# kazuto1011/dusty-gan

Measured on NVIDIA B200. Metric: chamfer_pairs_per_s, higher is better.
Workload: dtype f32

## Files before the change

### dusty-gan_b200/csrc/chamfer.cu

```cuda
#include <algorithm>

#include "common.cuh"

namespace dusty {
namespace chamfer {

constexpr int TPB = 256;
constexpr int TILE = 2048;
constexpr int CHUNK = 32;

struct Params {
  const float4* scanX;
  const float4* scanY;
  long long strideX, strideY;
  int countX, countY;
  int paddedX, paddedY;
  int row_begin, row_stride;
  int symmetric, mirror, compact_rows;
  float* M;
  long long ldm;
  float* dist1; float* dist2;
  int* idx1; int* idx2;
  const int2* metaX; const int2* metaY;
  const float4* boxX; const float4* boxY;
// ... 22 lines not shown

__device__ __forceinline__ float search_window(float ax, float ay, float az, float cur) {
  const float an = fmaf(az, az, fmaf(ax, ax, ay * ay));
  return fmaf(2.86102295e-6f , an + fmaxf(cur + an, 0.0f), 1e-36f);
}

template <bool WANT_INDEX>
__device__ __forceinline__ void warp_tile_exact_min(const float4* tp, int npairs, float ax, float ay, float az, int lane,
                                                    float& best, int& best_pos) {
  const f32x2 ax2 = pack2(ax, ax), ay2 = pack2(ay, ay), az2 = pack2(az, az);
  float e = __int_as_float(0x7f800000);
  int ei = 0x7fffffff;
  for (int q = lane; q < npairs; q += 32) {
    const float4 q0 = tp[2 * q], q1 = tp[2 * q + 1];
    const f32x2 dx = sub2(pack2(q0.x, q0.y), ax2);
    const f32x2 dy = sub2(pack2(q0.z, q0.w), ay2);
    const f32x2 dz = sub2(pack2(q1.x, q1.y), az2);
    float lo, hi;
    unpack2(fma2(dz, dz, fma2(dx, dx, mul2(dy, dy))), lo, hi);
    if (WANT_INDEX) {
      if (lo < e) { e = lo; ei = 2 * q; }
      if (hi < e) { e = hi; ei = 2 * q + 1; }
    } else {
      e = min3(e, lo, hi);
    }
  }
  float m = e;
  #pragma unroll
  for (int o = 16; o > 0; o >>= 1) m = fminf(m, __shfl_xor_sync(0xffffffffu, m, o));
  best = m;
  if (WANT_INDEX) {
    const bool mine = e == m && ei != 0x7fffffff;
    const unsigned key = mine ? (unsigned)ei : 0x7fffffffu;
    const unsigned kmin = __reduce_min_sync(0xffffffffu, key);
    const unsigned who = __ballot_sync(0xffffffffu, mine && key == kmin);
    best_pos = who ? __shfl_sync(0xffffffffu, ei, __ffs(who) - 1) : 0x7fffffff;
  }
}

template <bool WANT_INDEX>
__device__ __forceinline__ void warp_cloud_exact_min(const float4* cloud, int nchunks, const float4* boxes, float thr,
                                                     float ax, float ay, float az, int lane, const int* perm, float& best,
                                                     int& best_pos) {
  const f32x2 ax2 = pack2(ax, ax), ay2 = pack2(ay, ay), az2 = pack2(az, az);
  float e = __int_as_float(0x7f800000);
  int ei = 0x7fffffff;
  for (int ch = lane; ch < nchunks; ch += 32) {
    if (boxes != nullptr) {
      const float4 bl = boxes[2 * ch], bh = boxes[2 * ch + 1];
      const float gx = max3(0.0f, bl.x - ax, ax - bh.x), gy = max3(0.0f, bl.y - ay, ay - bh.y), gz = max3(0.0f, bl.z - az, az - bh.z);
      if (bl.w == 0.0f && fmaf(gz, gz, fmaf(gx, gx, __fmul_rn(gy, gy))) > thr) continue;
    }
    const float4* cp = cloud + (long long)ch * CHUNK;
    #pragma unroll 4
    for (int k = 0; k < CHUNK / 2; ++k) {
      const float4 q0 = cp[2 * k], q1 = cp[2 * k + 1];
      const f32x2 dx = sub2(pack2(q0.x, q0.y), ax2);
      const f32x2 dy = sub2(pack2(q0.z, q0.w), ay2);
      const f32x2 dz = sub2(pack2(q1.x, q1.y), az2);
      float lo, hi;
      unpack2(fma2(dz, dz, fma2(dx, dx, mul2(dy, dy))), lo, hi);
      if (WANT_INDEX) {
        const int i0 = ch * CHUNK + 2 * k;
        if (lo < e || (lo == e && ei != 0x7fffffff && (perm ? perm[i0] < perm[ei] : i0 < ei))) { e = lo; ei = i0; }
        if (hi < e || (hi == e && ei != 0x7fffffff && (perm ? perm[i0 + 1] < perm[ei] : i0 + 1 < ei))) { e = hi; ei = i0 + 1; }
      } else {
        e = min3(e, lo, hi);
      }
    }
  }
  float m = e;
  #pragma unroll
  for (int o = 16; o > 0; o >>= 1) m = fminf(m, __shfl_xor_sync(0xffffffffu, m, o));
  best = m;
  if (WANT_INDEX) {
    const bool mine = e == m && ei != 0x7fffffff;
    const unsigned key = mine ? (unsigned)(perm ? perm[ei] : ei) : 0x7fffffffu;
    const unsigned kmin = __reduce_min_sync(0xffffffffu, key);
    const unsigned who = __ballot_sync(0xffffffffu, mine && key == kmin);
    best_pos = who ? __shfl_sync(0xffffffffu, ei, __ffs(who) - 1) : 0x7fffffff;
  }
}

__device__ __forceinline__ void emit_entry(const Params& p, int ci, int cj, double S0, double S1) {
  const float v = (float)(S0 / (double)p.countX) + (float)(S1 / (double)p.countY);
  if (p.M) {
    p.M[(long long)(p.compact_rows ? (int)blockIdx.y : ci) * p.ldm + cj] = v;
    if (p.symmetric && p.mirror && ci != cj) p.M[(long long)cj * p.ldm + ci] = v;
  }
  if (p.keys) {
    const int gi = p.offX + ci, gj = p.offY + cj;
    if (gi != gj) {
      const unsigned long long vb = (unsigned long long)__float_as_uint(v) << 32;
      atomicMin(p.keys + gj, vb | (unsigned)gi);
      atomicMin(p.keys + gi, vb | (unsigned)gj);
      const int lo = min(gi, gj), hi = max(gi, gj);
      if (lo < p.n_ref && hi >= p.n_ref) {
        atomicMin(p.keys + p.n_total + hi, vb | (unsigned)lo);
        atomicMin(p.keys + 2 * (long long)p.n_total + lo, vb | (unsigned)hi);
      }
    }
  }
}

template <int R, bool MATRIX, bool MERGED, int NT = TPB>
__global__ void __launch_bounds__(NT, R >= 8 ? 512 / NT : (R == 4 ? 3 : 4)) nn_kernel(const Params p) {
  static_assert(!MERGED || MATRIX, "merged origins are a matrix front end layout");
  extern __shared__ __align__(128) unsigned char smem_raw[];
  float4* const tiles = reinterpret_cast<float4*>(smem_raw);
  __shared__ uint64_t bars[2];
  __shared__ double red[NT / 32];

  constexpr int RB = NT * R;
  constexpr int CH = (NT < TPB && !MERGED) ? CHUNK / 2 : CHUNK;
  constexpr int PR = CH / 2;
  const int tid = threadIdx.x;
  const int lane = tid & 31;

  int ci, cj;
  int dir_only = -1, rb_only = 0;
  if (MATRIX) {
    ci = p.row_begin + blockIdx.y * p.row_stride;
    cj = blockIdx.x;
    if (p.symmetric && cj < ci) return;
  } else {
    ci = cj = blockIdx.y;
    dir_only = blockIdx.z;
    rb_only = blockIdx.x;
    const int rows_here = dir_only == 0 ? p.countX : p.countY;
    if (rb_only >= (rows_here + RB - 1) / RB) return;
  }
  const float4* const sx = p.scanX + (long long)ci * p.strideX;
  const float4* const sy = p.scanY + (long long)cj * p.strideY;

  int2 mx = make_int2(p.countX, 1), my = make_int2(p.countY, 1);
  if (MERGED) { mx = p.metaX[ci]; my = p.metaY[cj]; }
#define K_ROW(r) (MERGED ? rb * RB + (tid >> 5) * (32 * R) + (r) * 32 + lane : rb * RB + (r) * NT + tid)
#define K_countX (MERGED ? mx.x : p.countX)
#define K_countY (MERGED ? my.x : p.countY)
#define K_paddedX (MERGED ? (mx.x + CHUNK - 1) / CHUNK * CHUNK : p.paddedX)
#define K_paddedY (MERGED ? (my.x + CHUNK - 1) / CHUNK * CHUNK : p.paddedY)

  const int ntX = (K_paddedX + TILE - 1) / TILE, ntY = (K_paddedY + TILE - 1) / TILE;
  const int nrbX = (K_countX + RB - 1) / RB, nrbY = (K_countY + RB - 1) / RB;
  const int seg0 = nrbX * ntY;
  int pos_begin, pos_end;
  if (MATRIX) { pos_begin = 0; pos_end = seg0 + nrbY * ntX; }
  else if (dir_only == 0) { pos_begin = rb_only * ntY; pos_end = pos_begin + ntY; }
  else { pos_begin = seg0 + rb_only * ntX; pos_end = pos_begin + ntX; }

  const int tstride = (R >= 8 && NT == TPB) ? TILE : min(TILE, max(p.paddedX, p.paddedY));
  if (tid == 0) { mbar_init(&bars[0], 1); mbar_init(&bars[1], 1); mbar_fence_init(); }
  __syncthreads();

  auto issue = [&](int pos, int buf) {
    int dir, t;
    if (pos < seg0) { dir = 0; t = pos % ntY; } else { dir = 1; t = (pos - seg0) % ntX; }
    const float4* src = (dir == 0 ? sy : sx) + (long long)t * TILE;
    const int padded = dir == 0 ? K_paddedY : K_paddedX;
    const int npts = min(TILE, padded - t * TILE);
    mbar_expect_tx(&bars[buf], (uint32_t)npts * 16u);
    bulk_g2s(tiles + buf * tstride, src, (uint32_t)npts * 16u, &bars[buf]);
  };
  if (tid == 0) issue(pos_begin, 0);

  f32x2 nax[R], nay[R], naz[R];
  float eb[R];
  int ei[R];
  float cur[R], sec[R];
  int cid[R];
// ... 128 lines not shown
        while (flagged) {
          const int src = __ffs(flagged) - 1;
          flagged &= flagged - 1;
          float m;
          int mi = 0;
          warp_tile_exact_min<!MATRIX>(tp, nch * PR, __shfl_sync(0xffffffffu, ax, src), __shfl_sync(0xffffffffu, ay, src),
                                       __shfl_sync(0xffffffffu, az, src), lane, m, mi);
          if (lane == src) {
            if (MATRIX) {
              eb[r] = fminf(eb[r], m);
            } else if (mi != 0x7fffffff) {
              mi += t * TILE;
              if (m < eb[r] || (m == eb[r] && mi < ei[r])) { eb[r] = m; ei[r] = mi; }
            }
          }
        }
      }
    }

    }

    if (MERGED && t == nt - 1 && rb * RB + (tid >> 5) * (32 * R) < rowcount) {
      const float4* const cand = dir == 0 ? sy : sx;
      #pragma unroll
      for (int r = 0; r < R; ++r) {
        float ax, ay, az, dummy;
        unpack2(nax[r], ax, dummy); unpack2(nay[r], ay, dummy); unpack2(naz[r], az, dummy);
        ax *= -0.5f; ay *= -0.5f; az *= -0.5f;
        const bool live = K_ROW(r) < rowcount;
        float e = __int_as_float(0x7f800000);
        if (live && cur[r] < __int_as_float(0x7f800000)) {
          const f32x2 ax2 = pack2(ax, ax), ay2 = pack2(ay, ay), az2 = pack2(az, az);
          const float4* cp = cand + (long long)cid[r] * CHUNK;
          #pragma unroll 4
          for (int k = 0; k < CHUNK / 2; ++k) {
            const float4 q0 = cp[2 * k], q1 = cp[2 * k + 1];
            const f32x2 dx = sub2(pack2(q0.x, q0.y), ax2);
            const f32x2 dy = sub2(pack2(q0.z, q0.w), ay2);
            const f32x2 dz = sub2(pack2(q1.x, q1.y), az2);
            float lo, hi;
            unpack2(fma2(dz, dz, fma2(dx, dx, mul2(dy, dy))), lo, hi);
            e = min3(e, lo, hi);
          }
        }
        eb[r] = e;
        const bool near_tie = live && sec[r] <= cur[r] + search_window(ax, ay, az, cur[r]);
        unsigned flagged = __ballot_sync(0xffffffffu, near_tie);
        while (flagged) {
          const int src = __ffs(flagged) - 1;
          flagged &= flagged - 1;
          float m;
          int mi;
          warp_cloud_exact_min<false>(cand, scanpadded / CHUNK, nullptr, 0.0f, __shfl_sync(0xffffffffu, ax, src),
                                      __shfl_sync(0xffffffffu, ay, src), __shfl_sync(0xffffffffu, az, src), lane, nullptr, m, mi);
          if (lane == src) eb[r] = fminf(eb[r], m);
        }
      }
    }

    if (t == nt - 1) {
      #pragma unroll
      for (int r = 0; r < R; ++r) {
        const int row = K_ROW(r);
        if (row < rowcount) {
          if (MATRIX) {
            if (MERGED) dsum += (row == rowcount - 1 ? (double)(dir == 0 ? mx.y : my.y) : 1.0) * (double)eb[r];
            else dsum += (double)eb[r];
          } else {
            float* dist = dir == 0 ? p.dist1 : p.dist2;
            int* idx = dir == 0 ? p.idx1 : p.idx2;
            const long long o = (long long)ci * rowcount + row;
            dist[o] = eb[r];
            if (idx) idx[o] = ei[r] == 0x7fffffff ? 0 : ei[r];
          }
        }
      }
    }
    if (MATRIX && pos == seg0 - 1) { S0 = block_sum<NT>(dsum, red); dsum = 0.0; }
    __syncthreads();
  }

  if (MATRIX) {
    const double S1 = block_sum<NT>(dsum, red);
    if (tid == 0) emit_entry(p, ci, cj, S0, S1);
  }
}

#undef K_ROW
#undef K_countX
#undef K_countY
#undef K_paddedX
#undef K_paddedY

__global__ void __launch_bounds__(256) prep_kernel(const float* __restrict__ xyz, long long clouds, int count,
                                                   int padded, float4* __restrict__ out) {
  const long long half = padded / 2;
  const long long g = (long long)blockIdx.x * blockDim.x + threadIdx.x;
  if (g >= clouds * half) return;
  const long long c = g / half;
  const int q = (int)(g - c * half);
  const float nan = __int_as_float(0x7fc00000);
  float v[2][4];
  #pragma unroll
  for (int s = 0; s < 2; ++s) {
    const int pt = 2 * q + s;
    if (pt < count) {
      const float* src = xyz + (c * count + pt) * 3;
      const float x = src[0], y = src[1], z = src[2];
      v[s][0] = x; v[s][1] = y; v[s][2] = z;
      v[s][3] = fmaf(z, z, fmaf(x, x, y * y));
    } else {
      v[s][0] = v[s][1] = v[s][2] = v[s][3] = nan;
    }
  }
  out[g * 2] = make_float4(v[0][0], v[1][0], v[0][1], v[1][1]);
  out[g * 2 + 1] = make_float4(v[0][2], v[1][2], v[0][3], v[1][3]);
}

__global__ void __launch_bounds__(256) prep_merge_kernel(const float* __restrict__ xyz, int count, long long stride,
                                                         float4* __restrict__ out, int2* __restrict__ meta) {
  __shared__ int wsum[8];
  const long long c = blockIdx.x;
  const int tid = threadIdx.x, lane = tid & 31, warp = tid >> 5;
  const float* src = xyz + c * count * 3;
  float* dst = reinterpret_cast<float*>(out + c * stride);
  const int per = (count + 255) / 256;
  const int begin = min(tid * per, count), end = min(begin + per, count);
  int mine = 0;
  for (int i = begin; i < end; ++i) mine += (src[3 * i] != 0.0f) || (src[3 * i + 1] != 0.0f) || (src[3 * i + 2] != 0.0f);
  int inc = mine;
  #pragma unroll
  for (int o = 1; o < 32; o <<= 1) { const int t = __shfl_up_sync(0xffffffffu, inc, o); if (lane >= o) inc += t; }
  if (lane == 31) wsum[warp] = inc;
  __syncthreads();
  int before = 0, total = 0;
  #pragma unroll
  for (int w = 0; w < 8; ++w) { if (w < warp) before += wsum[w]; total += wsum[w]; }
  auto put = [&](int pos, float x, float y, float z, float n) {
    float* q = dst + (size_t)(pos >> 1) * 8 + (pos & 1);
    q[0] = x; q[2] = y; q[4] = z; q[6] = n;
  };
  int pos = before + inc - mine;
  for (int i = begin; i < end; ++i) {
    const float x = src[3 * i], y = src[3 * i + 1], z = src[3 * i + 2];
    if (x != 0.0f || y != 0.0f || z != 0.0f) put(pos++, x, y, z, fmaf(z, z, fmaf(x, x, y * y)));
  }
  const int zeros = count - total;
  const int kept = total + (zeros > 0 ? 1 : 0);
  if (tid == 0) {
    if (zeros > 0) put(total, 0.0f, 0.0f, 0.0f, 0.0f);
    meta[c] = make_int2(kept, zeros > 0 ? zeros : 1);
  }
  const float nan = __int_as_float(0x7fc00000);
  const int padded = (kept + CHUNK - 1) / CHUNK * CHUNK;
  for (int i = kept + tid; i < padded; i += 256) put(i, nan, nan, nan, nan);
}

constexpr int SORT_CAP = 32768;
constexpr int SORT_TPB = 1024;
constexpr int WALK_BLOCKS = SORT_CAP / CHUNK / 32;

__device__ __forceinline__ unsigned spread7(unsigned v) {
  v &= 0x7fu;
  v = (v | (v << 4)) & 0x070fu;
  v = (v | (v << 2)) & 0x1333u;
  v = (v | (v << 1)) & 0x1555u;
  return v;
// ... 649 lines not shown
```

### dusty-gan_b200/csrc/chamfer_pair.cuh

```cuda
constexpr int PAIR_CAP = 2048;
constexpr int PAIR_NW = 8;

__global__ void __launch_bounds__(PAIR_NW * 32, 3) nn_pair_split_kernel(const Params p) {
  constexpr int SUB = 8;
  constexpr int GR = 32;
  extern __shared__ __align__(128) unsigned char smem_raw[];
  __shared__ uint64_t bar;
  __shared__ double tsum[2 * (PAIR_CAP / GR)];
  __shared__ int next_task;
  const int tid = threadIdx.x, lane = tid & 31;
  const int h = lane >> 4, l16 = lane & 15;

  const int ci = p.row_begin + blockIdx.y * p.row_stride;
  const int cj = blockIdx.x;
  if (p.symmetric && cj < ci) return;

  const int2 mx = p.metaX[ci], my = p.metaY[cj];
  const int padX = (mx.x + CHUNK - 1) / CHUNK * CHUNK, padY = (my.x + CHUNK - 1) / CHUNK * CHUNK;
  float4* const sX = reinterpret_cast<float4*>(smem_raw);
  float4* const sY = sX + p.paddedX;
  float4* const bX = sY + p.paddedY;
  float4* const bY = bX + p.paddedX / CHUNK * 2;
  if (tid == 0) {
    mbar_init(&bar, 1);
    mbar_fence_init();
    next_task = 0;
    const uint32_t bytes = (uint32_t)(padX + padY) * 16u + (uint32_t)(padX / CHUNK + padY / CHUNK) * 32u;
    mbar_expect_tx(&bar, bytes);
    bulk_g2s(sX, p.scanX + (long long)ci * p.strideX, (uint32_t)padX * 16u, &bar);
    bulk_g2s(sY, p.scanY + (long long)cj * p.strideY, (uint32_t)padY * 16u, &bar);
    bulk_g2s(bX, p.boxX + (long long)ci * (p.paddedX / CHUNK * 2), (uint32_t)(padX / CHUNK) * 32u, &bar);
    bulk_g2s(bY, p.boxY + (long long)cj * (p.paddedY / CHUNK * 2), (uint32_t)(padY / CHUNK) * 32u, &bar);
  }
  __syncthreads();
  mbar_wait(&bar, 0);

  const int ngX = (mx.x + GR - 1) / GR, ngY = (my.x + GR - 1) / GR;
  const float inf = __int_as_float(0x7f800000);

  for (;;) {
    int task = 0;
    if (lane == 0) task = atomicAdd(&next_task, 1);
    task = __shfl_sync(0xffffffffu, task, 0);
    if (task >= ngX + ngY) break;
    const int dir = task >= ngX;
    const int g = dir ? task - ngX : task;
    const float4* const rows = dir ? sY : sX;
    const float4* const cand = dir ? sX : sY;
    const float4* const rbox = dir ? bY : bX;
    const float4* const cbox = dir ? bX : bY;
    const int rowcount = dir ? my.x : mx.x;
    const int nch = (dir ? padX : padY) / CHUNK;

    f32x2 nax[2], nay[2], naz[2];
    float cur[2], sec[2];
    int cid[2];
    float rx[2], ry[2], rz[2];
    #pragma unroll
    for (int j = 0; j < 2; ++j) {
      const int row = g * GR + j * 16 + l16;
      const int rr = row < rowcount ? row : 0;
      const float* f = reinterpret_cast<const float*>(rows + (rr >> 1) * 2) + (rr & 1);
      rx[j] = f[0]; ry[j] = f[2]; rz[j] = f[4];
      const float mx2 = -2.0f * rx[j], my2 = -2.0f * ry[j], mz2 = -2.0f * rz[j];
      nax[j] = pack2(mx2, mx2); nay[j] = pack2(my2, my2); naz[j] = pack2(mz2, mz2);
      cur[j] = sec[j] = inf; cid[j] = 0;
    }
    const float oax = h ? rx[1] : rx[0], oay = h ? ry[1] : ry[0], oaz = h ? rz[1] : rz[0];
    const float an = fmaf(oaz, oaz, fmaf(oax, oax, oay * oay));
    const int orow = g * GR + lane;
    float ubr = orow < rowcount ? inf : -1.0f;
    float gl0, gl1, gl2, gh0, gh1, gh2;
    {
      const float4 bl = rbox[2 * g], bh = rbox[2 * g + 1];
      gl0 = bl.x; gl1 = bl.y; gl2 = bl.z; gh0 = bh.x; gh1 = bh.y; gh2 = bh.z;
      if (bl.w != 0.0f) {
        gl0 = fminf(gl0, 0.0f); gl1 = fminf(gl1, 0.0f); gl2 = fminf(gl2, 0.0f);
        gh0 = fmaxf(gh0, 0.0f); gh1 = fmaxf(gh1, 0.0f); gh2 = fmaxf(gh2, 0.0f);
      }
    }
    const bool forced = cbox[2 * (nch - 1)].w != 0.0f;
    unsigned key[2];
    #pragma unroll
    for (int q = 0; q < 2; ++q) {
      const int c = q * 32 + lane;
      key[q] = 0xffffffffu;
      if (forced && c == nch - 1) {
        key[q] = (unsigned)c;
      } else if (c < nch) {
        const float4 bl = cbox[2 * c], bh = cbox[2 * c + 1];
        const float gx = max3(0.0f, bl.x - gh0, gl0 - bh.x), gy = max3(0.0f, bl.y - gh1, gl1 - bh.y), gz = max3(0.0f, bl.z - gh2, gl2 - bh.z);
        const float lb = fmaf(gz, gz, fmaf(gx, gx, __fmul_rn(gy, gy)));
        if (lb < inf) key[q] = (__float_as_uint(lb) & ~63u) | (unsigned)c;
      }
    }
    float ubmax = inf;
    int nvis = 0;
    for (;;) {
      const unsigned kwin = __reduce_min_sync(0xffffffffu, min(key[0], key[1]));
      if (kwin == 0xffffffffu) break;
      if (__uint_as_float(kwin & ~63u) > ubmax) break;
      const int c = (int)(kwin & 63u);
      if (key[0] == kwin) key[0] = 0xffffffffu;
      if (key[1] == kwin) key[1] = 0xffffffffu;
      const float4 bl = cbox[2 * c], bh = cbox[2 * c + 1];
      const float qx = max3(0.0f, bl.x - oax, oax - bh.x), qy = max3(0.0f, bl.y - oay, oay - bh.y), qz = max3(0.0f, bl.z - oaz, oaz - bh.z);
      const bool need = (forced && c == nch - 1) || fmaf(qz, qz, fmaf(qx, qx, __fmul_rn(qy, qy))) <= ubr;
      if (!__any_sync(0xffffffffu, need)) continue;
      ++nvis;
      const float4* cp = cand + c * CHUNK + h * (CHUNK / 2);
      #pragma unroll
      for (int w = 0; w < 2; ++w) {
        float cm[2];
        #pragma unroll
        for (int k = w * 4; k < w * 4 + 4; ++k) {
          const float4 q0 = cp[2 * k], q1 = cp[2 * k + 1];
          const f32x2 bx = pack2(q0.x, q0.y), by = pack2(q0.z, q0.w);
          const f32x2 bz = pack2(q1.x, q1.y), bn = pack2(q1.z, q1.w);
          #pragma unroll
          for (int j = 0; j < 2; ++j) {
            f32x2 s = fma2(naz[j], bz, bn);
            s = fma2(nay[j], by, s);
            s = fma2(nax[j], bx, s);
            float lo, hi;
            unpack2(s, lo, hi);
            cm[j] = (k == w * 4) ? fminf(lo, hi) : min3(cm[j], lo, hi);
          }
        }
        const int wid = c * (CHUNK / SUB) + 2 * h + w;
        #pragma unroll
        for (int j = 0; j < 2; ++j) {
          const bool better = cm[j] < cur[j];
          sec[j] = fminf(sec[j], better ? cur[j] : cm[j]);
          cur[j] = fminf(cur[j], cm[j]);
          cid[j] = better ? wid : cid[j];
        }
      }
      const float other = __shfl_xor_sync(0xffffffffu, h ? cur[0] : cur[1], 16);
      if (ubr >= 0.0f) {
        const float dest = fmaxf(fminf(h ? cur[1] : cur[0], other) + an, 0.0f);
        ubr = fmaf(3.81469727e-6f , an + dest, dest) + 1e-36f;
      }
      ubmax = __uint_as_float(__reduce_max_sync(0xffffffffu, __float_as_uint(fmaxf(ubr, 0.0f))));
    }
    if (p.visited != nullptr && lane == 0)
      atomicAdd(p.visited, (unsigned long long)nvis * CHUNK * (unsigned long long)min(GR, rowcount - g * GR));

    const float pc = __shfl_xor_sync(0xffffffffu, h ? cur[0] : cur[1], 16);
    const float ps = __shfl_xor_sync(0xffffffffu, h ? sec[0] : sec[1], 16);
    const int pi = __shfl_xor_sync(0xffffffffu, h ? cid[0] : cid[1], 16);
    const float mc = h ? cur[1] : cur[0], ms = h ? sec[1] : sec[0];
    const int mi0 = h ? cid[1] : cid[0];
    const bool theirs = pc < mc;
    const float c1 = fminf(mc, pc);
    const float s1 = fminf(fminf(ms, ps), theirs ? mc : pc);
    const int w1 = theirs ? pi : mi0;
    const bool live = orow < rowcount;
    float e = inf;
    if (live && c1 < inf) {
      const f32x2 ax2 = pack2(oax, oax), ay2 = pack2(oay, oay), az2 = pack2(oaz, oaz);
      const float4* cp = cand + w1 * SUB;
      #pragma unroll
      for (int k = 0; k < SUB / 2; ++k) {
        const int kk = (k + lane) & (SUB / 2 - 1);
        const float4 q0 = cp[2 * kk], q1 = cp[2 * kk + 1];
        const f32x2 dx = sub2(pack2(q0.x, q0.y), ax2);
        const f32x2 dy = sub2(pack2(q0.z, q0.w), ay2);
        const f32x2 dz = sub2(pack2(q1.x, q1.y), az2);
        float lo, hi;
        unpack2(fma2(dz, dz, fma2(dx, dx, mul2(dy, dy))), lo, hi);
        e = min3(e, lo, hi);
      }
    }
    const bool near_tie = live && s1 <= c1 + search_window(oax, oay, oaz, c1);
    unsigned flagged = __ballot_sync(0xffffffffu, near_tie);
    while (flagged) {
      const int src = __ffs(flagged) - 1;
      flagged &= flagged - 1;
      float m;
      int mi;
      warp_cloud_exact_min<false>(cand, nch, cbox, __shfl_sync(0xffffffffu, e, src), __shfl_sync(0xffffffffu, oax, src),
                                  __shfl_sync(0xffffffffu, oay, src), __shfl_sync(0xffffffffu, oaz, src), lane, nullptr, m, mi);
      if (lane == src) e = fminf(e, m);
    }
    double dsum = live ? (orow == rowcount - 1 ? (double)(dir ? my.y : mx.y) : 1.0) * (double)e : 0.0;
    #pragma unroll
    for (int o = 16; o > 0; o >>= 1) dsum += __shfl_down_sync(0xffffffffu, dsum, o);
    if (lane == 0) tsum[task] = dsum;
  }

  __syncthreads();
  if (tid == 0) {
    double S0 = 0.0, S1 = 0.0;
    for (int t = 0; t < ngX; ++t) S0 += tsum[t];
    for (int t = ngX; t < ngX + ngY; ++t) S1 += tsum[t];
    emit_entry(p, ci, cj, S0, S1);
  }
}

static int launch_pair_split(const Params& p, dim3 grid, cudaStream_t st) {
  const size_t smem = (size_t)(p.paddedX + p.paddedY) * 16 + (size_t)(p.paddedX / CHUNK + p.paddedY / CHUNK) * 32;
  static bool configured[kMaxDevices] = {};
  const int dev = current_device();
  if (!configured[dev]) {
    DUSTY_CUDA(cudaFuncSetAttribute(nn_pair_split_kernel, cudaFuncAttributeMaxDynamicSharedMemorySize,
                                    2 * PAIR_CAP * 16 + 2 * (PAIR_CAP / CHUNK) * 32));
    configured[dev] = true;
  }
  nn_pair_split_kernel<<<grid, PAIR_NW * 32, smem, st>>>(p);
  DUSTY_AFTER_LAUNCH("chamfer nn_pair_split_kernel");
  return 0;
}
```

### dusty-gan_b200/csrc/chamfer_walk.cuh

```cuda
constexpr int WALK_NW = 8;
constexpr int WALK_TPC = 8;
constexpr int WALK_SPLIT_MAXTASKS = 2 * (SORT_CAP / 32 + 1);

template <bool MATRIX>
__global__ void __launch_bounds__(WALK_NW * 32, 3) nn_walk_split_kernel(const Params p) {
  constexpr int SUB = 8;
  constexpr int GR = 32;
  __shared__ double tsum[MATRIX ? WALK_SPLIT_MAXTASKS : 1];
  __shared__ int next_task;
  __shared__ float4 stage[WALK_NW][CHUNK];
  const int tid = threadIdx.x, lane = tid & 31;
  const int h = lane >> 4, l16 = lane & 15;
  int ci, cj;
  if (MATRIX) {
    ci = p.row_begin + blockIdx.y * p.row_stride;
    cj = blockIdx.x;
    if (p.symmetric && cj < ci) return;
  } else {
    ci = cj = blockIdx.y;
  }
  const int2 mx = p.metaX[ci], my = p.metaY[cj];
  const int padX = (mx.x + CHUNK - 1) / CHUNK * CHUNK, padY = (my.x + CHUNK - 1) / CHUNK * CHUNK;
  const float4* const sX = p.scanX + (long long)ci * p.strideX;
  const float4* const sY = p.scanY + (long long)cj * p.strideY;
// ... 114 lines not shown
            sec[j] = fminf(sec[j], better ? cur[j] : cm[j]);
            cur[j] = fminf(cur[j], cm[j]);
            cid[j] = better ? wid : cid[j];
          }
        }
        const float other = __shfl_xor_sync(0xffffffffu, h ? cur[0] : cur[1], 16);
        if (ubr >= 0.0f) {
          const float dest = fmaxf(fminf(h ? cur[1] : cur[0], other) + an, 0.0f);
          ubr = fmaf(3.81469727e-6f , an + dest, dest) + 1e-36f;
        }
        ubmax = __uint_as_float(__reduce_max_sync(0xffffffffu, __float_as_uint(fmaxf(ubr, 0.0f))));
      }
    }
    if (p.visited != nullptr && lane == 0)
      atomicAdd(p.visited, (unsigned long long)nvis * CHUNK * (unsigned long long)min(GR, rowcount - g * GR));

    const float pc = __shfl_xor_sync(0xffffffffu, h ? cur[0] : cur[1], 16);
    const float ps = __shfl_xor_sync(0xffffffffu, h ? sec[0] : sec[1], 16);
    const int pi = __shfl_xor_sync(0xffffffffu, h ? cid[0] : cid[1], 16);
    const float mc = h ? cur[1] : cur[0], ms = h ? sec[1] : sec[0];
    const int mi0 = h ? cid[1] : cid[0];
    const bool theirs = pc < mc;
    const float c1 = fminf(mc, pc);
    const float s1 = fminf(fminf(ms, ps), theirs ? mc : pc);
    const int w1 = theirs ? pi : mi0;
    const bool live = orow < rowcount;
    float e = inf;
    int eidx = 0x7fffffff;
    if (live && c1 < inf) {
      const f32x2 ax2 = pack2(oax, oax), ay2 = pack2(oay, oay), az2 = pack2(oaz, oaz);
      const float4* cp = cand + (long long)w1 * SUB;
      #pragma unroll
      for (int k = 0; k < SUB / 2; ++k) {
        const float4 q0 = __ldg(cp + 2 * k), q1 = __ldg(cp + 2 * k + 1);
        const f32x2 dx = sub2(pack2(q0.x, q0.y), ax2);
        const f32x2 dy = sub2(pack2(q0.z, q0.w), ay2);
        const f32x2 dz = sub2(pack2(q1.x, q1.y), az2);
        float lo, hi;
        unpack2(fma2(dz, dz, fma2(dx, dx, mul2(dy, dy))), lo, hi);
        if (MATRIX) {
          e = min3(e, lo, hi);
        } else {
          const int i0 = w1 * SUB + 2 * k;
          if (lo < e || (lo == e && eidx != 0x7fffffff && cperm[i0] < cperm[eidx])) { e = lo; eidx = i0; }
          if (hi < e || (hi == e && eidx != 0x7fffffff && cperm[i0 + 1] < cperm[eidx])) { e = hi; eidx = i0 + 1; }
        }
      }
    }
    const bool near_tie = live && s1 <= c1 + search_window(oax, oay, oaz, c1);
    unsigned flagged = __ballot_sync(0xffffffffu, near_tie);
    while (flagged) {
      const int src = __ffs(flagged) - 1;
      flagged &= flagged - 1;
      float m;
      int mi = 0x7fffffff;
      warp_cloud_exact_min<!MATRIX>(cand, nch, cbox, __shfl_sync(0xffffffffu, e, src), __shfl_sync(0xffffffffu, oax, src),
                                    __shfl_sync(0xffffffffu, oay, src), __shfl_sync(0xffffffffu, oaz, src), lane, cperm, m, mi);
      if (lane == src) {
        if (MATRIX) {
          e = fminf(e, m);
        } else if (mi != 0x7fffffff && (m < e || (m == e && (eidx == 0x7fffffff || cperm[mi] < cperm[eidx])))) {
          e = m; eidx = mi;
        }
      }
    }
    if (MATRIX) {
      double dsum = live ? (orow == rowcount - 1 ? (double)(dir ? my.y : mx.y) : 1.0) * (double)e : 0.0;
      #pragma unroll
      for (int o = 16; o > 0; o >>= 1) dsum += __shfl_down_sync(0xffffffffu, dsum, o);
      if (lane == 0) tsum[task] = dsum;
    } else if (live) {
      const long long o = (long long)ci * (dir ? p.strideY : p.strideX) + orow;
      (dir ? p.dist2 : p.dist1)[o] = e;
      (dir ? p.idx2 : p.idx1)[o] = cperm[eidx == 0x7fffffff ? 0 : eidx];
    }
  }

  if (MATRIX) {
    __syncthreads();
    if (tid == 0) {
      double S0 = 0.0, S1 = 0.0;
      for (int t = 0; t < ngX; ++t) S0 += tsum[t];
      for (int t = ngX; t < ngX + ngY; ++t) S1 += tsum[t];
      emit_entry(p, ci, cj, S0, S1);
    }
  }
}

template <bool MATRIX>
static int launch_walk_split(const Params& p, dim3 grid, cudaStream_t st) {
  nn_walk_split_kernel<MATRIX><<<grid, WALK_NW * 32, 0, st>>>(p);
  DUSTY_AFTER_LAUNCH("chamfer nn_walk_split_kernel");
  return 0;
}
```

### dusty-gan_b200/csrc/common.cuh

```cuda
#pragma once

#include <cuda_runtime.h>
#include <stdint.h>
#include <stddef.h>

#include "dusty_b200.h"

namespace dusty {

int fail_cuda(cudaError_t e, const char* what);
int fail_arg(int code, const char* fmt, ...);
void count_launches(int n);
int check_device();
int current_device();
constexpr int kMaxDevices = 64;

constexpr int kNumSMs = 148;

inline size_t align_up(size_t v, size_t a) { return (v + a - 1) / a * a; }
inline bool aligned16(const void* p) { return (reinterpret_cast<uintptr_t>(p) & 15u) == 0; }

#define DUSTY_CUDA(call)                                                    \
  do {                                                                      \
    cudaError_t e__ = (call);                                               \
    if (e__ != cudaSuccess) return ::dusty::fail_cuda(e__, #call);          \
  } while (0)

#define DUSTY_AFTER_LAUNCH(name)                                            \
  do {                                                                      \
    ::dusty::count_launches(1);                                             \
    cudaError_t e__ = cudaGetLastError();                                   \
    if (e__ != cudaSuccess) return ::dusty::fail_cuda(e__, name);           \
  } while (0)

#ifdef __CUDACC__

typedef unsigned long long f32x2;

__device__ __forceinline__ f32x2 pack2(float lo, float hi) {
  f32x2 r; asm("mov.b64 %0, {%1, %2};" : "=l"(r) : "f"(lo), "f"(hi)); return r;
}
__device__ __forceinline__ void unpack2(f32x2 v, float& lo, float& hi) {
  asm("mov.b64 {%0, %1}, %2;" : "=f"(lo), "=f"(hi) : "l"(v));
}
__device__ __forceinline__ f32x2 fma2(f32x2 a, f32x2 b, f32x2 c) {
  f32x2 d; asm("fma.rn.f32x2 %0, %1, %2, %3;" : "=l"(d) : "l"(a), "l"(b), "l"(c)); return d;
}
__device__ __forceinline__ f32x2 mul2(f32x2 a, f32x2 b) {
  f32x2 d; asm("mul.rn.f32x2 %0, %1, %2;" : "=l"(d) : "l"(a), "l"(b)); return d;
}
__device__ __forceinline__ f32x2 sub2(f32x2 a, f32x2 b) {
  f32x2 d; asm("sub.rn.f32x2 %0, %1, %2;" : "=l"(d) : "l"(a), "l"(b)); return d;
}
__device__ __forceinline__ float min3(float a, float b, float c) {
  float d; asm("min.f32 %0, %1, %2, %3;" : "=f"(d) : "f"(a), "f"(b), "f"(c)); return d;
}
__device__ __forceinline__ float max3(float a, float b, float c) {
  float d; asm("max.f32 %0, %1, %2, %3;" : "=f"(d) : "f"(a), "f"(b), "f"(c)); return d;
}

__device__ __forceinline__ uint32_t smem_u32(const void* p) {
  return static_cast<uint32_t>(__cvta_generic_to_shared(p));
}
__device__ __forceinline__ void mbar_init(uint64_t* bar, uint32_t count) {
  asm volatile("mbarrier.init.shared::cta.b64 [%0], %1;" ::"r"(smem_u32(bar)), "r"(count) : "memory");
}
__device__ __forceinline__ void mbar_fence_init() {
  asm volatile("fence.mbarrier_init.release.cluster;" ::: "memory");
}
__device__ __forceinline__ void mbar_expect_tx(uint64_t* bar, uint32_t bytes) {
  asm volatile("mbarrier.arrive.expect_tx.shared::cta.b64 _, [%0], %1;" ::"r"(smem_u32(bar)), "r"(bytes) : "memory");
}
__device__ __forceinline__ void mbar_wait(uint64_t* bar, uint32_t parity) {
  asm volatile(
      "{\n\t"
      ".reg .pred p;\n\t"
      "WAIT_%=:\n\t"
      "mbarrier.try_wait.parity.shared::cta.b64 p, [%0], %1;\n\t"
      "@p bra DONE_%=;\n\t"
      "bra WAIT_%=;\n\t"
      "DONE_%=:\n\t"
      "}" ::"r"(smem_u32(bar)), "r"(parity) : "memory");
}
__device__ __forceinline__ void bulk_g2s(void* smem_dst, const void* gmem_src, uint32_t bytes, uint64_t* bar) {
  asm volatile("cp.async.bulk.shared::cluster.global.mbarrier::complete_tx::bytes [%0], [%1], %2, [%3];" ::"r"(
                   smem_u32(smem_dst)),
               "l"(gmem_src), "r"(bytes), "r"(smem_u32(bar))
               : "memory");
}

__device__ __forceinline__ float4 ldg_stream(const float4* p) {
  float4 r;
  asm volatile("ld.global.nc.L1::no_allocate.v4.f32 {%0,%1,%2,%3}, [%4];"
               : "=f"(r.x), "=f"(r.y), "=f"(r.z), "=f"(r.w) : "l"(p));
  return r;
}
__device__ __forceinline__ void stg_stream(float4* p, const float4& v) {
  asm volatile("st.global.L1::no_allocate.v4.f32 [%0], {%1,%2,%3,%4};" ::"l"(p), "f"(v.x), "f"(v.y), "f"(v.z), "f"(v.w) : "memory");
}

#endif

}
```

Baseline: 7.659 million.

## Compact symmetric pair grid and streamline chunk walk in pair split kernel

For symmetric inputs, the pair kernel now launches only the upper-triangle blocks. Each block maps its linear index back to (row slot, column) with a sqrt-based inverse plus a correction loop, so blocks that would exit at once are no longer launched. The chunk walk is also reworked: keys are pre-sorted per lane and the next winner is reduced ahead of time, box tests use packed f32x2 subtraction, and the two SUB windows are merged with a NaN-propagating max for the runner-up. The changes aim to cut wasted CTA launches and per-iteration instruction count, at the cost of index-decode math and some subtle changes to runner-up tracking.

```diff
diff --git a/dusty-gan_b200/csrc/chamfer.cu b/dusty-gan_b200/csrc/chamfer.cu
--- a/dusty-gan_b200/csrc/chamfer.cu
+++ b/dusty-gan_b200/csrc/chamfer.cu
@@ -128,10 +128,10 @@
   }
 }
 
-__device__ __forceinline__ void emit_entry(const Params& p, int ci, int cj, double S0, double S1) {
+__device__ __forceinline__ void emit_entry(const Params& p, int slot, int ci, int cj, double S0, double S1) {
   const float v = (float)(S0 / (double)p.countX) + (float)(S1 / (double)p.countY);
   if (p.M) {
-    p.M[(long long)(p.compact_rows ? (int)blockIdx.y : ci) * p.ldm + cj] = v;
+    p.M[(long long)(p.compact_rows ? slot : ci) * p.ldm + cj] = v;
     if (p.symmetric && p.mirror && ci != cj) p.M[(long long)cj * p.ldm + ci] = v;
   }
   if (p.keys) {
@@ -426,7 +426,7 @@
 
   if (MATRIX) {
     const double S1 = block_sum<NT>(dsum, red);
-    if (tid == 0) emit_entry(p, ci, cj, S0, S1);
+    if (tid == 0) emit_entry(p, (int)blockIdx.y, ci, cj, S0, S1);
   }
 }
 
diff --git a/dusty-gan_b200/csrc/chamfer_pair.cuh b/dusty-gan_b200/csrc/chamfer_pair.cuh
--- a/dusty-gan_b200/csrc/chamfer_pair.cuh
+++ b/dusty-gan_b200/csrc/chamfer_pair.cuh
@@ -1,7 +1,20 @@
 constexpr int PAIR_CAP = 2048;
 constexpr int PAIR_NW = 8;
 
-__global__ void __launch_bounds__(PAIR_NW * 32, 3) nn_pair_split_kernel(const Params p) {
+__host__ __device__ __forceinline__ long long pair_tri_prefix(long long k, int ncols, int row_begin, int row_stride) {
+  return k * (ncols - row_begin) - (long long)row_stride * (k * (k - 1) / 2);
+}
+
+__device__ __forceinline__ void pair_tri_entry(long long b, int ncols, int row_begin, int row_stride, int& k, int& cj) {
+  const double a = (double)(ncols - row_begin) + 0.5 * row_stride;
+  long long r = (long long)((a - sqrt(fmax(a * a - 2.0 * row_stride * (double)b, 0.0))) / row_stride);
+  while (r > 0 && pair_tri_prefix(r, ncols, row_begin, row_stride) > b) --r;
+  while (pair_tri_prefix(r + 1, ncols, row_begin, row_stride) <= b) ++r;
+  k = (int)r;
+  cj = row_begin + k * row_stride + (int)(b - pair_tri_prefix(r, ncols, row_begin, row_stride));
+}
+
+__global__ void __launch_bounds__(PAIR_NW * 32, 3) nn_pair_split_kernel(const Params p, int ncols, long long tri) {
   constexpr int SUB = 8;
   constexpr int GR = 32;
   extern __shared__ __align__(128) unsigned char smem_raw[];
@@ -9,11 +22,18 @@
   __shared__ double tsum[2 * (PAIR_CAP / GR)];
   __shared__ int next_task;
   const int tid = threadIdx.x, lane = tid & 31;
-  const int h = lane >> 4, l16 = lane & 15;
-
-  const int ci = p.row_begin + blockIdx.y * p.row_stride;
-  const int cj = blockIdx.x;
-  if (p.symmetric && cj < ci) return;
+  const int h = lane >> 4;
+
+  int slot, cj;
+  if (p.symmetric) {
+    const long long b = (long long)blockIdx.y * gridDim.x + blockIdx.x;
+    if (b >= tri) return;
+    pair_tri_entry(b, ncols, p.row_begin, p.row_stride, slot, cj);
+  } else {
+    slot = blockIdx.y;
+    cj = blockIdx.x;
+  }
+  const int ci = p.row_begin + slot * p.row_stride;
 
   const int2 mx = p.metaX[ci], my = p.metaY[cj];
   const int padX = (mx.x + CHUNK - 1) / CHUNK * CHUNK, padY = (my.x + CHUNK - 1) / CHUNK * CHUNK;
@@ -40,7 +60,8 @@
 
   for (;;) {
     int task = 0;
-    if (lane == 0) task = atomicAdd(&next_task, 1);
+    if (lane == 0)
+      asm volatile("atom.shared.add.u32 %0, [%1], 1;" : "=r"(task) : "r"(smem_u32(&next_task)) : "memory");
     task = __shfl_sync(0xffffffffu, task, 0);
     if (task >= ngX + ngY) break;
     const int dir = task >= ngX;
@@ -56,9 +77,10 @@
     float cur[2], sec[2];
     int cid[2];
     float rx[2], ry[2], rz[2];
+    const int orow = g * GR + lane;
     #pragma unroll
     for (int j = 0; j < 2; ++j) {
-      const int row = g * GR + j * 16 + l16;
+      const int row = orow ^ (j * 16);
       const int rr = row < rowcount ? row : 0;
       const float* f = reinterpret_cast<const float*>(rows + (rr >> 1) * 2) + (rr & 1);
       rx[j] = f[0]; ry[j] = f[2]; rz[j] = f[4];
@@ -66,54 +88,65 @@
       nax[j] = pack2(mx2, mx2); nay[j] = pack2(my2, my2); naz[j] = pack2(mz2, mz2);
       cur[j] = sec[j] = inf; cid[j] = 0;
     }
-    const float oax = h ? rx[1] : rx[0], oay = h ? ry[1] : ry[0], oaz = h ? rz[1] : rz[0];
+    const float oax = rx[0], oay = ry[0], oaz = rz[0];
+    const f32x2 oaxy = pack2(oax, oay);
     const float an = fmaf(oaz, oaz, fmaf(oax, oax, oay * oay));
-    const int orow = g * GR + lane;
-    float ubr = orow < rowcount ? inf : -1.0f;
-    float gl0, gl1, gl2, gh0, gh1, gh2;
+    const bool live = orow < rowcount;
+    float ubr = live ? inf : -1.0f;
+    f32x2 gl01, gh01;
+    float gl2, gh2;
     {
       const float4 bl = rbox[2 * g], bh = rbox[2 * g + 1];
-      gl0 = bl.x; gl1 = bl.y; gl2 = bl.z; gh0 = bh.x; gh1 = bh.y; gh2 = bh.z;
+      float gl0 = bl.x, gl1 = bl.y, gh0 = bh.x, gh1 = bh.y;
+      gl2 = bl.z; gh2 = bh.z;
       if (bl.w != 0.0f) {
         gl0 = fminf(gl0, 0.0f); gl1 = fminf(gl1, 0.0f); gl2 = fminf(gl2, 0.0f);
         gh0 = fmaxf(gh0, 0.0f); gh1 = fmaxf(gh1, 0.0f); gh2 = fmaxf(gh2, 0.0f);
       }
-    }
-    const bool forced = cbox[2 * (nch - 1)].w != 0.0f;
+      gl01 = pack2(gl0, gl1); gh01 = pack2(gh0, gh1);
+    }
+    const int cforced = cbox[2 * (nch - 1)].w != 0.0f ? nch - 1 : -1;
     unsigned key[2];
     #pragma unroll
     for (int q = 0; q < 2; ++q) {
       const int c = q * 32 + lane;
       key[q] = 0xffffffffu;
-      if (forced && c == nch - 1) {
+      if (c == cforced) {
         key[q] = (unsigned)c;
       } else if (c < nch) {
         const float4 bl = cbox[2 * c], bh = cbox[2 * c + 1];
-        const float gx = max3(0.0f, bl.x - gh0, gl0 - bh.x), gy = max3(0.0f, bl.y - gh1, gl1 - bh.y), gz = max3(0.0f, bl.z - gh2, gl2 - bh.z);
+        float dlx, dly, dhx, dhy;
+        unpack2(sub2(pack2(bl.x, bl.y), gh01), dlx, dly);
+        unpack2(sub2(gl01, pack2(bh.x, bh.y)), dhx, dhy);
+        const float gx = max3(0.0f, dlx, dhx), gy = max3(0.0f, dly, dhy), gz = max3(0.0f, bl.z - gh2, gl2 - bh.z);
         const float lb = fmaf(gz, gz, fmaf(gx, gx, __fmul_rn(gy, gy)));
         if (lb < inf) key[q] = (__float_as_uint(lb) & ~63u) | (unsigned)c;
       }
     }
+    {
+      const unsigned k0 = min(key[0], key[1]), k1 = max(key[0], key[1]);
+      key[0] = k0; key[1] = k1;
+    }
+    const float4* const candh = cand + h * (CHUNK / 2);
     float ubmax = inf;
     int nvis = 0;
-    for (;;) {
-      const unsigned kwin = __reduce_min_sync(0xffffffffu, min(key[0], key[1]));
-      if (kwin == 0xffffffffu) break;
-      if (__uint_as_float(kwin & ~63u) > ubmax) break;
+    unsigned kwin = __reduce_min_sync(0xffffffffu, key[0]);
+    while (kwin != 0xffffffffu && __uint_as_float(kwin & ~63u) <= ubmax) {
       const int c = (int)(kwin & 63u);
-      if (key[0] == kwin) key[0] = 0xffffffffu;
-      if (key[1] == kwin) key[1] = 0xffffffffu;
+      if (key[0] == kwin) { key[0] = key[1]; key[1] = 0xffffffffu; }
+      const unsigned knext = __reduce_min_sync(0xffffffffu, key[0]);
       const float4 bl = cbox[2 * c], bh = cbox[2 * c + 1];
-      const float qx = max3(0.0f, bl.x - oax, oax - bh.x), qy = max3(0.0f, bl.y - oay, oay - bh.y), qz = max3(0.0f, bl.z - oaz, oaz - bh.z);
-      const bool need = (forced && c == nch - 1) || fmaf(qz, qz, fmaf(qx, qx, __fmul_rn(qy, qy))) <= ubr;
-      if (!__any_sync(0xffffffffu, need)) continue;
-      ++nvis;
-      const float4* cp = cand + c * CHUNK + h * (CHUNK / 2);
-      #pragma unroll
-      for (int w = 0; w < 2; ++w) {
-        float cm[2];
+      float dlx, dly, dhx, dhy;
+      unpack2(sub2(pack2(bl.x, bl.y), oaxy), dlx, dly);
+      unpack2(sub2(oaxy, pack2(bh.x, bh.y)), dhx, dhy);
+      const float qx = max3(0.0f, dlx, dhx), qy = max3(0.0f, dly, dhy), qz = max3(0.0f, bl.z - oaz, oaz - bh.z);
+      const bool need = c == cforced || fmaf(qz, qz, fmaf(qx, qx, __fmul_rn(qy, qy))) <= ubr;
+      if (__any_sync(0xffffffffu, need)) {
+        ++nvis;
+        const float4* const cp = candh + c * CHUNK;
+        float cm[2][2];
         #pragma unroll
-        for (int k = w * 4; k < w * 4 + 4; ++k) {
+        for (int k = 0; k < 8; ++k) {
           const float4 q0 = cp[2 * k], q1 = cp[2 * k + 1];
           const f32x2 bx = pack2(q0.x, q0.y), by = pack2(q0.z, q0.w);
           const f32x2 bz = pack2(q1.x, q1.y), bn = pack2(q1.z, q1.w);
@@ -124,38 +157,40 @@
             s = fma2(nax[j], bx, s);
             float lo, hi;
             unpack2(s, lo, hi);
-            cm[j] = (k == w * 4) ? fminf(lo, hi) : min3(cm[j], lo, hi);
+            cm[k >> 2][j] = (k & 3) == 0 ? fminf(lo, hi) : min3(cm[k >> 2][j], lo, hi);
           }
         }
-        const int wid = c * (CHUNK / SUB) + 2 * h + w;
+        const int wid = c * (CHUNK / SUB) + 2 * h;
         #pragma unroll
         for (int j = 0; j < 2; ++j) {
-          const bool better = cm[j] < cur[j];
-          sec[j] = fminf(sec[j], better ? cur[j] : cm[j]);
-          cur[j] = fminf(cur[j], cm[j]);
-          cid[j] = better ? wid : cid[j];
+          const float c0 = cm[0][j], c1 = cm[1][j];
+          const float mn = fminf(c0, c1);
+          const bool better = mn < cur[j];
+          sec[j] = min3(sec[j], maxnan(cur[j], mn), maxnan(c0, c1));
+          cur[j] = fminf(cur[j], mn);
+          cid[j] = better ? wid + (c1 < c0) : cid[j];
         }
-      }
-      const float other = __shfl_xor_sync(0xffffffffu, h ? cur[0] : cur[1], 16);
-      if (ubr >= 0.0f) {
-        const float dest = fmaxf(fminf(h ? cur[1] : cur[0], other) + an, 0.0f);
-        ubr = fmaf(3.81469727e-6f , an + dest, dest) + 1e-36f;
-      }
-      ubmax = __uint_as_float(__reduce_max_sync(0xffffffffu, __float_as_uint(fmaxf(ubr, 0.0f))));
+        const float other = __shfl_xor_sync(0xffffffffu, cur[1], 16);
+        if (live) {
+          const float dest = fmaxf(fminf(cur[0], other) + an, 0.0f);
+          ubr = fmaf(3.81469727e-6f , an + dest, dest) + 1e-36f;
+        }
+        ubmax = __int_as_float(__reduce_max_sync(0xffffffffu, __float_as_int(ubr)));
+      }
+      kwin = knext;
     }
     if (p.visited != nullptr && lane == 0)
       atomicAdd(p.visited, (unsigned long long)nvis * CHUNK * (unsigned long long)min(GR, rowcount - g * GR));
 
-    const float pc = __shfl_xor_sync(0xffffffffu, h ? cur[0] : cur[1], 16);
-    const float ps = __shfl_xor_sync(0xffffffffu, h ? sec[0] : sec[1], 16);
-    const int pi = __shfl_xor_sync(0xffffffffu, h ? cid[0] : cid[1], 16);
-    const float mc = h ? cur[1] : cur[0], ms = h ? sec[1] : sec[0];
-    const int mi0 = h ? cid[1] : cid[0];
+    const float pc = __shfl_xor_sync(0xffffffffu, cur[1], 16);
+    const float ps = __shfl_xor_sync(0xffffffffu, sec[1], 16);
+    const int pi = __shfl_xor_sync(0xffffffffu, cid[1], 16);
+    const float mc = cur[0], ms = sec[0];
+    const int mi0 = cid[0];
     const bool theirs = pc < mc;
     const float c1 = fminf(mc, pc);
     const float s1 = fminf(fminf(ms, ps), theirs ? mc : pc);
     const int w1 = theirs ? pi : mi0;
-    const bool live = orow < rowcount;
     float e = inf;
     if (live && c1 < inf) {
       const f32x2 ax2 = pack2(oax, oax), ay2 = pack2(oay, oay), az2 = pack2(oaz, oaz);
@@ -194,11 +229,18 @@
     double S0 = 0.0, S1 = 0.0;
     for (int t = 0; t < ngX; ++t) S0 += tsum[t];
     for (int t = ngX; t < ngX + ngY; ++t) S1 += tsum[t];
-    emit_entry(p, ci, cj, S0, S1);
+    emit_entry(p, slot, ci, cj, S0, S1);
   }
 }
 
 static int launch_pair_split(const Params& p, dim3 grid, cudaStream_t st) {
+  const int ncols = (int)grid.x;
+  long long tri = 0;
+  if (p.symmetric) {
+    tri = pair_tri_prefix(grid.y, ncols, p.row_begin, p.row_stride);
+    const long long gx = std::min(tri, 1ll << 24);
+    grid = dim3((unsigned)gx, (unsigned)((tri + gx - 1) / gx), 1);
+  }
   const size_t smem = (size_t)(p.paddedX + p.paddedY) * 16 + (size_t)(p.paddedX / CHUNK + p.paddedY / CHUNK) * 32;
   static bool configured[kMaxDevices] = {};
   const int dev = current_device();
@@ -207,7 +249,7 @@
                                     2 * PAIR_CAP * 16 + 2 * (PAIR_CAP / CHUNK) * 32));
     configured[dev] = true;
   }
-  nn_pair_split_kernel<<<grid, PAIR_NW * 32, smem, st>>>(p);
+  nn_pair_split_kernel<<<grid, PAIR_NW * 32, smem, st>>>(p, ncols, tri);
   DUSTY_AFTER_LAUNCH("chamfer nn_pair_split_kernel");
   return 0;
 }
diff --git a/dusty-gan_b200/csrc/chamfer_walk.cuh b/dusty-gan_b200/csrc/chamfer_walk.cuh
--- a/dusty-gan_b200/csrc/chamfer_walk.cuh
+++ b/dusty-gan_b200/csrc/chamfer_walk.cuh
@@ -220,7 +220,7 @@
       double S0 = 0.0, S1 = 0.0;
       for (int t = 0; t < ngX; ++t) S0 += tsum[t];
       for (int t = ngX; t < ngX + ngY; ++t) S1 += tsum[t];
-      emit_entry(p, ci, cj, S0, S1);
+      emit_entry(p, (int)blockIdx.y, ci, cj, S0, S1);
     }
   }
 }
diff --git a/dusty-gan_b200/csrc/common.cuh b/dusty-gan_b200/csrc/common.cuh
--- a/dusty-gan_b200/csrc/common.cuh
+++ b/dusty-gan_b200/csrc/common.cuh
@@ -59,6 +59,10 @@
   float d; asm("max.f32 %0, %1, %2, %3;" : "=f"(d) : "f"(a), "f"(b), "f"(c)); return d;
 }
 
+__device__ __forceinline__ float maxnan(float a, float b) {
+  float d; asm("max.NaN.f32 %0, %1, %2;" : "=f"(d) : "f"(a), "f"(b)); return d;
+}
+
 __device__ __forceinline__ uint32_t smem_u32(const void* p) {
   return static_cast<uint32_t>(__cvta_generic_to_shared(p));
 }
diff --git a/profiles/sass_pair_phases.py b/profiles/sass_pair_phases.py
--- /dev/null
+++ b/profiles/sass_pair_phases.py
@@ -0,0 +1,96 @@
+import collections
+import glob
+import os
+import re
+import subprocess
+import sys
+import tempfile
+
+ROOT = os.path.dirname(os.path.dirname(os.path.abspath(__file__)))
+LIB = os.path.join(ROOT, "dusty-gan_b200", "lib", "libdustyb200.so")
+SRC = os.path.join(ROOT, "dusty-gan_b200", "csrc", "chamfer_pair.cuh")
+KERNEL = "_ZN5dusty7chamfer20nn_pair_split_kernel"
+PHASES = [
+    ("CTA prologue (entry, TMA, barrier)", "CTA", ["nn_pair_split_kernel(const Params p"]),
+    ("task set-up (fetch, rows, -2x, leaf box)", "group", ["int task = 0;"]),
+    ("key build (two chunk keys per lane)", "group", ["const bool forced = cbox", "const int cforced = cbox"]),
+    ("pick + point-to-box test + vote", "pick", ["float ubmax = inf;", "kwin = knext;"]),
+    ("scan body (LDS, FFMA2, FMNMX3)", "chunk", ["++nvis;"]),
+    ("window tracking (min, runner-up, id)", "chunk", ["const int wid = c * (CHUNK / SUB)"]),
+    ("bound update (shuffle, ubr, REDUX.MAX)", "chunk", ["// bound of the lane's own row"]),
+    ("visited-pairs counter", "group", ["if (p.visited != nullptr"]),
+    ("merge + exact pass on the winning window", "group", ["// ---- merge the halves"]),
+    ("near-tie guard", "group", ["const bool near_tie"]),
+    ("dsum reduction", "group", ["double dsum"]),
+    ("CTA finish (task sums, emit_entry)", "CTA", ["double S0 = 0.0"]),
+]
+OPS = ["FFMA2", "FMNMX", "LDS", "SHFL", "REDUX", "VOTE", "FADD", "FSEL", "SEL", "ISETP", "FSETP", "BRA"]
+
+
+def line_phases():
+    src = open(SRC).read().split("\n")
+    starts = []
+    for name, unit, anchors in PHASES:
+        for i, text in enumerate(src, 1):
+            if any(a in text for a in anchors):
+                starts.append((i, name))
+    starts.sort()
+    return lambda ln: ([n for i, n in starts if i <= ln] or [PHASES[0][0]])[-1]
+
+
+def disassemble():
+    with tempfile.TemporaryDirectory() as tmp:
+        subprocess.run(["cuobjdump", "-xelf", "all", LIB], cwd=tmp, check=True, capture_output=True)
+        for cubin in sorted(glob.glob(os.path.join(tmp, "*.cubin"))):
+            names = subprocess.run(["cuobjdump", "-symbols", cubin], capture_output=True, text=True).stdout
+            if KERNEL in names:
+                res = subprocess.run(["cuobjdump", "-res-usage", cubin], capture_output=True, text=True).stdout
+                return subprocess.run(["nvdisasm", "-gi", cubin], capture_output=True, text=True, check=True).stdout, res
+    sys.exit("nn_pair_split_kernel not found in " + LIB)
+
+
+def main():
+    text, res = disassemble()
+    body = text[text.index("\n.text." + KERNEL):]
+    body = body[:body.find("\n//----")]
+    phase_of = line_phases()
+    insts = []
+    where = None
+    for raw in body.split("\n"):
+        locs = re.findall(r'"([^"]+)", line (\d+)', raw)
+        if raw.lstrip().startswith("//## File") and locs:
+            where = locs[-1]
+            continue
+        m = re.match(r"\s+/\*[0-9a-f]{4,}\*/\s+(@!?U?P\w+\s+)?([A-Z0-9_.]+)", raw)
+        if m:
+            on_pair = where is not None and where[0].endswith("chamfer_pair.cuh")
+            insts.append((phase_of(int(where[1])) if on_pair else "other", m.group(2), m.group(2) == "EXIT" and not m.group(1)))
+    last_exit = max(i for i, (_, _, plain) in enumerate(insts) if plain)
+    counts = collections.OrderedDict((name, collections.Counter()) for name, _, _ in PHASES)
+    counts["other"] = collections.Counter()
+    counts["cold copies after the last EXIT"] = collections.Counter()
+    for i, (phase, op, _) in enumerate(insts):
+        key = phase if i <= last_exit else "cold copies after the last EXIT"
+        c = counts[key]
+        c["all"] += 1
+        c[next((o for o in OPS if op == o or op.startswith(o + ".") or (o == "REDUX" and op.startswith("CREDUX"))), "rest")] += 1
+    unit = {name: u for name, u, _ in PHASES}
+    regs = re.search(KERNEL + r".*?\n.*?REG:(\d+).*?SHARED:(\d+)", res, re.S)
+    out = ["nn_pair_split_kernel: SASS instructions per phase (static; python profiles/sass_pair_phases.py)",
+           "registers %s, static shared memory %s bytes (dynamic: 2 x 32 KB clouds + 2 x 1 KB boxes at 2048 points)"
+           % (regs.group(1), regs.group(2)) if regs else "", "",
+           "%-44s %-6s %6s " % ("phase", "runs", "instrs") + " ".join("%6s" % o for o in OPS + ["rest"])]
+    for name, c in counts.items():
+        if c["all"]:
+            out.append("%-44s %-6s %6d " % (name, unit.get(name, ""), c["all"]) + " ".join("%6d" % c[o] for o in OPS + ["rest"]))
+    per_chunk = sum(counts[n]["all"] for n, u, _ in PHASES if u == "chunk")
+    per_pick = sum(counts[n]["all"] for n, u, _ in PHASES if u == "pick")
+    per_group = sum(counts[n]["all"] for n, u, _ in PHASES if u == "group")
+    out += ["", "per scanned chunk %d, per pick %d, per group outside the walk %d, kernel total %d (hot %d)"
+            % (per_chunk, per_pick, per_group, len(insts), last_exit + 1)]
+    open(os.path.join(ROOT, "profiles", "sass_pair_phases.txt"), "w").write("\n".join(out) + "\n")
+    print("\n".join(out))
+
+
+if __name__ == "__main__":
+    main()
```

New measurement: 7.818 million, median of 6. 2.1% higher.
